# genomematt/xenomapper

Measured on AMD Instinct MI355X. Metric: read-pairs/sec classified, higher is better.
Workload: dtype int32; 1 GPU; configs[1]: 50000000 PE 2x150 pairs/GPU, AS/XS, liberal, HBM-resident; pairs_per_gpu=50000000, step=xm_classify_compact_dev: classify+count, scan, scatter (3 launches)

## Files before the change

### xenomapper_amd/csrc/xm_api.hip

```cpp
#include <hip/hip_runtime.h>
#include <stdint.h>
#include <stdio.h>
#include <stdlib.h>
#include <string.h>

#include <dlfcn.h>

#include <string>
#include <vector>

#include <rccl/rccl.h>

#include "xm_kernels.h"
#include "xm_pinned.h"

struct TimedSpan {
    int kernel;
    hipEvent_t start, stop;
};

namespace {

enum Scratch {
    S_COL0, S_COL1, S_COL2, S_COL3,
// ... 123 lines not shown
        launch();
    }
    return check_launch(ctx, what);
}

int drain_spans(xm_ctx *ctx)
{
    for (auto &sp : ctx->spans) {
        XM_HIP(ctx, hipEventSynchronize(sp.stop));
        float ms = 0.f;
        XM_HIP(ctx, hipEventElapsedTime(&ms, sp.start, sp.stop));
        ctx->acc_ms[sp.kernel] += (double)ms;
        ctx->acc_launches[sp.kernel] += 1;
        ctx->free_events.push_back(sp.start);
        ctx->free_events.push_back(sp.stop);
    }
    ctx->spans.clear();
    return XM_OK;
}

const size_t COUNTS_REP_BYTES = (XM_COUNT_REPLICAS * 64 + 8) * sizeof(uint64_t);
const size_t PART_TOT_BYTES = (size_t)XM_PART_REPLICAS * 8 * XM_PART_STRIDE * sizeof(uint32_t);

void reset_count_state(xm_ctx *ctx, hipStream_t st)
{
    (void)hipMemsetAsync(ctx->d_counts_rep, 0, COUNTS_REP_BYTES, st);
    (void)hipMemsetAsync(ctx->d_part_tot, 0, PART_TOT_BYTES, st);
}

void free_workspace(xm_ctx *ctx)
{
    if (ctx->d_gran_counts) (void)hipFree(ctx->d_gran_counts);
    if (ctx->d_gran_off) (void)hipFree(ctx->d_gran_off);
    if (ctx->d_counts_rep) (void)hipFree(ctx->d_counts_rep);
    if (ctx->d_part_tot) (void)hipFree(ctx->d_part_tot);
    if (ctx->ws_event) (void)hipEventDestroy(ctx->ws_event);
}

bool bad_mode(int mode) { return mode < XM_MODE_SE || mode > XM_MODE_PE_CONSERVATIVE; }

bool wrong_device(const xm_ctx *ctx)
{
    int cur = -1;
    return hipGetDevice(&cur) != hipSuccess || cur != ctx->device;
}

bool bad_call(const xm_ctx *ctx, int mode, uint64_t n) { return !ctx || bad_mode(mode) || n > XM_MAX_RECORDS; }
bool bad_dev_call(const xm_ctx *ctx, int mode, uint64_t n) { return bad_call(ctx, mode, n) || wrong_device(ctx); }

template <typename... P>
bool misaligned(uintptr_t mask, P... p) { return ((... | (uintptr_t)p) & mask) != 0; }

bool bad_totals(const uint64_t *offsets, const uint64_t *counts) { return !offsets || !counts || misaligned(7u, offsets, counts); }

bool capturing(hipStream_t st)
{
    hipStreamCaptureStatus cs = hipStreamCaptureStatusNone;
    if (hipStreamIsCapturing(st, &cs) != hipSuccess) { (void)hipGetLastError(); return false; }
    return cs != hipStreamCaptureStatusNone;
}

int order_workspace(xm_ctx *ctx, hipStream_t st)
{
    if (capturing(st)) return XM_OK;
    if (ctx->ws_released) {
        XM_HIP(ctx, hipStreamWaitEvent(st, ctx->ws_event, 0));
        ctx->ws_released = false;
    } else if (ctx->ws_used && ctx->ws_stream != st && !capturing(ctx->ws_stream)) {
        XM_HIP(ctx, hipEventRecord(ctx->ws_event, ctx->ws_stream));
        XM_HIP(ctx, hipStreamWaitEvent(st, ctx->ws_event, 0));
    }
    ctx->ws_stream = st;
    ctx->ws_used = true;
    return XM_OK;
}


template <typename T>
struct ScoreCols {
    const T *as1, *xs1, *as2, *xs2;
    const uint64_t *unit_bits;
    T min_score;
    static constexpr bool chunkable = true;
    static const char *kernel_name(bool counting)
    {
        if (sizeof(T) == sizeof(int32_t)) return counting ? "classify_kernel<int32, counts>" : "classify_kernel<int32>";
        return counting ? "classify_kernel<f64, counts>" : "classify_kernel<f64>";
    }
    bool missing() const { return !as1 || !xs1 || !as2 || !xs2 || !unit_bits; }
    bool misplaced() const { return misaligned(4 * sizeof(T) - 1, as1, xs1, as2, xs2) || misaligned(7u, unit_bits); }
    void classify(hipStream_t st, int mode, uint64_t n, uint8_t *code_out, const xm::CountPlan *cp) const
    {
        xm::launch_classify<T>(st, mode, n, as1, xs1, as2, xs2, unit_bits, min_score, code_out, cp);
    }
};

struct PackedCols {
    xm::CigCols s1, s2;
    const uint64_t *unit_bits;
    int32_t min_score_floor;
    uint32_t *range_flag;
    static constexpr bool chunkable = false;
    static const char *kernel_name(bool) { return "classify_cigp_kernel"; }
    bool missing() const
    {
        return !s1.nm || !s1.cnt || !s1.tile || !s1.ops || !s1.xs || !s2.nm || !s2.cnt || !s2.tile || !s2.ops || !s2.xs || !unit_bits;
    }
    bool misplaced() const
    {
        return misaligned(15u, s1.nm, s1.xs, s2.nm, s2.xs) || misaligned(7u, unit_bits) ||
               misaligned(3u, s1.cnt, s2.cnt, s1.tile, s2.tile, s1.ops, s2.ops, range_flag);
    }
    void classify(hipStream_t st, int mode, uint64_t n, uint8_t *code_out, const xm::CountPlan *cp) const
    {
        xm::launch_classify_cigp(st, mode, n, s1, s2, unit_bits, min_score_floor, code_out, range_flag, *cp);
    }
};


template <typename T>
int classify_dev(xm_ctx *ctx, hipStream_t st, int mode, uint64_t n, const ScoreCols<T> &in, uint8_t *code_out)
{
    if (bad_dev_call(ctx, mode, n)) return XM_ERR_INVALID_ARG;
    if (n == 0) return XM_OK;
    if (in.missing() || !code_out) return XM_ERR_INVALID_ARG;
    if (in.misplaced() || misaligned(3u, code_out)) return XM_ERR_INVALID_ARG;
    return timed_launch(ctx, st, XM_K_CLASSIFY, in.kernel_name(false), [&] { in.classify(st, mode, n, code_out, nullptr); });
}

int compact_tail(xm_ctx *ctx, hipStream_t st, int mode, uint64_t n, const uint8_t *code, const xm::CountPlan &cp,
                 uint32_t *idx_out, uint64_t *bin_offsets, uint64_t *counts, const xm::ListOut *lists = nullptr)
{
    const bool from_bins4 = cp.bins4 != nullptr;
    uint64_t *bin_totals = ctx->d_counts_rep + XM_COUNT_REPLICAS * 64;
    int rc = timed_launch(ctx, st, XM_K_SCAN, "scan_kernel", [&] {
        xm::launch_scan(st, cp, ctx->d_gran_off, bin_totals, counts);
    });
    if (rc == XM_OK)
        rc = timed_launch(ctx, st, XM_K_SCATTER, "scatter_kernel", [&] {
            xm::launch_scatter(st, cp.plan, mode, n, from_bins4 ? cp.bins4 : code, from_bins4, cp.gran_counts, ctx->d_gran_off,
                               bin_totals, bin_offsets, idx_out, ctx->d_part_tot, lists, cp.gran0, cp.gran1);
        });
    if (rc != XM_OK) reset_count_state(ctx, st);
    return rc;
}

xm::CountPlan count_plan(xm_ctx *ctx, uint64_t n)
{
    xm::CountPlan cp;
    cp.plan = xm::plan_granules(n);
    cp.gran_counts = ctx->d_gran_counts;
    cp.counts_rep = ctx->d_counts_rep;
    cp.part_tot = ctx->d_part_tot;
    return cp;
}

int empty_compact(xm_ctx *ctx, hipStream_t st, uint64_t *bin_offsets, uint64_t *counts)
{
    XM_HIP(ctx, hipMemsetAsync(counts, 0, 64 * sizeof(uint64_t), st));
    XM_HIP(ctx, hipMemsetAsync(bin_offsets, 0, 8 * sizeof(uint64_t), st));
    return XM_OK;
}


struct FusedDest {
    bool six_lists;
    uint32_t *flat;
    uint32_t *const *six;
    uint32_t *state6;
    uint64_t capacity;
};
FusedDest flat_list(uint32_t *idx_out) { return {false, idx_out, nullptr, nullptr, 0}; }
FusedDest six_lists(uint32_t *const idx_out[6], uint32_t *idx_state6, uint64_t cap) { return {true, nullptr, idx_out, idx_state6, cap}; }

int list_out(const FusedDest &to, xm::ListOut &lo)
{
    if (!to.six) return XM_ERR_INVALID_ARG;
    for (int b = 0; b < 6; ++b) {
        if (!to.six[b] || misaligned(3u, to.six[b])) return XM_ERR_INVALID_ARG;
        lo.p[b] = to.six[b];
    }
    if (misaligned(3u, to.state6)) return XM_ERR_INVALID_ARG;
    lo.p[6] = to.state6;
    lo.cap = to.capacity > 0xFFFFFFFFull ? 0xFFFFFFFFu : (uint32_t)to.capacity;
    return XM_OK;
}

uint32_t place_chunk_granules(void)
{
    const char *e = getenv("XM_PLACE_CHUNK_PARTS");
    const long v = e && *e ? strtol(e, nullptr, 10) : 0;
    return (uint32_t)(v < 0 ? 0 : v > 2048 ? 2048 : v) * (uint32_t)XM_PART_GRAN;
}

template <typename In>
int place_steps(xm_ctx *ctx, hipStream_t st, int mode, uint64_t n, const In &in, xm::CountPlan &cp, uint8_t *code_out,
                uint32_t *idx_out, const xm::ListOut *lists, uint64_t *totals, uint64_t *counts, bool may_chunk)
{
    const uint32_t n_gran = cp.plan.n_gran, chunk = may_chunk ? place_chunk_granules() : 0u;
    const bool chunked = chunk != 0u && n_gran > 2u * chunk;
    int rc;
    for (uint32_t g0 = 0; g0 < n_gran; g0 += chunked ? chunk : n_gran) {
        if (chunked) {
            cp.gran0 = g0;
            cp.gran1 = n_gran - g0 > chunk ? g0 + chunk : n_gran;
        }
        rc = timed_launch(ctx, st, XM_K_CLASSIFY, in.kernel_name(true), [&] { in.classify(st, mode, n, code_out, &cp); });
        if (rc != XM_OK) {
            if (g0) reset_count_state(ctx, st);
            return rc;
        }
        if ((rc = compact_tail(ctx, st, mode, n, code_out, cp, idx_out, totals, counts, lists)) != XM_OK) return rc;
    }
    return XM_OK;
}

template <typename In>
int fused_step(xm_ctx *ctx, hipStream_t st, int mode, uint64_t n, const In &in, uint8_t *code_out, uint8_t *bins4,
               const FusedDest &to, uint64_t *totals, uint64_t *counts)
{
    if (bad_dev_call(ctx, mode, n)) return XM_ERR_INVALID_ARG;
    if (bad_totals(totals, counts)) return XM_ERR_INVALID_ARG;
    xm::ListOut lo;
    int rc;
    if (to.six_lists && (rc = list_out(to, lo)) != XM_OK) return rc;
    if (n == 0) return empty_compact(ctx, st, totals, counts);
    if (in.missing() || (!code_out && !bins4) || (!to.six_lists && !to.flat)) return XM_ERR_INVALID_ARG;
    if (in.misplaced() || misaligned(15u, code_out, bins4) || misaligned(3u, to.flat)) return XM_ERR_INVALID_ARG;
    xm::CountPlan cp = count_plan(ctx, n);
    cp.bins4 = bins4;
    if ((rc = order_workspace(ctx, st)) != XM_OK) return rc;
    return place_steps(ctx, st, mode, n, in, cp, code_out, to.flat, to.six_lists ? &lo : nullptr, totals, counts,
                       In::chunkable && to.six_lists);
}


template <typename T>
int classify_runs(xm_ctx *ctx, hipStream_t st, int mode, uint64_t n, const ScoreCols<T> &in,
                  uint16_t *runs16, uint16_t *gran_counts, uint64_t *n_out, uint64_t *counts)
{
    if (bad_dev_call(ctx, mode, n)) return XM_ERR_INVALID_ARG;
    if (bad_totals(n_out, counts)) return XM_ERR_INVALID_ARG;
    if (n == 0) return empty_compact(ctx, st, n_out, counts);
    if (in.missing() || !runs16 || !gran_counts) return XM_ERR_INVALID_ARG;
    if (in.misplaced() || misaligned(15u, runs16, gran_counts)) return XM_ERR_INVALID_ARG;
    const xm::RunsOut ro = {runs16, gran_counts, ctx->d_counts_rep};
    int rc;
    if ((rc = order_workspace(ctx, st)) != XM_OK) return rc;
    rc = timed_launch(ctx, st, XM_K_CLASSIFY, "classify_runs_kernel", [&] {
        xm::launch_classify_runs<T>(st, mode, n, in.as1, in.xs1, in.as2, in.xs2, in.unit_bits, in.min_score, ro);
    });
    if (rc != XM_OK) return rc;
    rc = timed_launch(ctx, st, XM_K_SCAN, "runs_finish_kernel", [&] {
        xm::launch_runs_finish(st, mode, ctx->d_counts_rep, counts, n_out);
    });
    if (rc != XM_OK) reset_count_state(ctx, st);
    return rc;
}


template <typename T>
int upload_score_cols(xm_ctx *ctx, uint64_t n, const ScoreCols<T> &host, ScoreCols<T> &dev)
{
    const size_t col_bytes = (size_t)n * sizeof(T);
    const size_t bits_bytes = (size_t)((n + 63) / 64) * 8;
    const T *src[4] = {host.as1, host.xs1, host.as2, host.xs2};
    int rc;
    for (int c = 0; c < 4; ++c) {
        if ((rc = ensure_scratch(ctx, S_COL0 + c, col_bytes)) != XM_OK) return rc;
        XM_HIP(ctx, hipMemcpy(ctx->d_scratch[S_COL0 + c], src[c], col_bytes, hipMemcpyHostToDevice));
    }
    if ((rc = ensure_scratch(ctx, S_BITS, bits_bytes)) != XM_OK) return rc;
    XM_HIP(ctx, hipMemcpy(ctx->d_scratch[S_BITS], host.unit_bits, bits_bytes, hipMemcpyHostToDevice));
    dev = {(const T *)ctx->d_scratch[S_COL0], (const T *)ctx->d_scratch[S_COL1], (const T *)ctx->d_scratch[S_COL2],
           (const T *)ctx->d_scratch[S_COL3], (const uint64_t *)ctx->d_scratch[S_BITS], host.min_score};
    return XM_OK;
}

int ensure_code_scratch(xm_ctx *ctx, uint64_t n, bool want_bytes, uint8_t *&d_code, uint8_t *&d_bins4)
{
    const int rc = ensure_scratch(ctx, S_CODE, want_bytes ? (size_t)n + 16 : (size_t)XM_BINS4_BYTES(n));
    d_code = want_bytes ? (uint8_t *)ctx->d_scratch[S_CODE] : nullptr;
    d_bins4 = want_bytes ? nullptr : (uint8_t *)ctx->d_scratch[S_CODE];
    return rc;
}

int fetch_results(xm_ctx *ctx, uint64_t n, int n_lists, int word0, const uint32_t *const d_list[], uint32_t *const list[],
                  uint64_t cap, uint8_t *code_out, uint64_t totals[8], uint64_t counts[64])
{
    uint64_t host[72];
    XM_HIP(ctx, hipMemcpy(host, ctx->d_scratch[S_TOTALS], sizeof host, hipMemcpyDeviceToHost));
    memcpy(totals, host, 8 * sizeof(uint64_t));
    if (counts) memcpy(counts, host + 8, 64 * sizeof(uint64_t));
    for (int b = 0; b < n_lists; ++b) {
        const uint64_t k = host[word0 + b] < cap ? host[word0 + b] : cap;
        if (k) XM_HIP(ctx, hipMemcpy(list[b], d_list[b], (size_t)k * 4, hipMemcpyDeviceToHost));
    }
    if (code_out) XM_HIP(ctx, hipMemcpy(code_out, ctx->d_scratch[S_CODE], (size_t)n, hipMemcpyDeviceToHost));
    return XM_OK;
}

int fetch_compact_results(xm_ctx *ctx, uint64_t n, uint8_t *code_out, uint32_t *idx_out, uint64_t bin_offsets[8], uint64_t counts[64])
{
    const uint32_t *d_idx = (const uint32_t *)ctx->d_scratch[S_IDX];
    return fetch_results(ctx, n, 1, 7, &d_idx, &idx_out, n, code_out, bin_offsets, counts);
}

int counts_only_tail(xm_ctx *ctx, const xm::CountPlan &cp, uint64_t *d_counts)
{
    xm::launch_scan(nullptr, cp, ctx->d_gran_off, ctx->d_counts_rep + XM_COUNT_REPLICAS * 64, d_counts);
    const int rc = check_launch(ctx, "scan_kernel");
    if (rc != XM_OK) reset_count_state(ctx, nullptr);
    else (void)hipMemsetAsync(ctx->d_part_tot, 0, PART_TOT_BYTES, nullptr);
// ... 834 lines not shown
```

### xenomapper_amd/csrc/xm_kernels.h

```cpp
#pragma once
#include <hip/hip_runtime.h>
#include <stdint.h>

#include "../../include/xenomapper_hip.h"

#define XM_BLOCK 256
#define XM_GRAN 2048
#define XM_MAX_GRANULES ((uint32_t)((0xFFFFF000ull + XM_GRAN - 1) / XM_GRAN))
#define XM_PART_GRAN 1024u
#define XM_PART_STRIDE 2112u
#define XM_PART_REPLICAS 64u
#define XM_COUNT_REPLICAS 64u
#define XM_CLASSIFY_BLOCK 512
#ifndef XM_CIGAR_BLOCK
#define XM_CIGAR_BLOCK 256
#endif
#define XM_CIGP_BLOCK 512
#ifndef XM_SCATTER_WAVES
#define XM_SCATTER_WAVES 1048576u
#endif
#define XM_CLASSIFY_NT true

namespace xm {

struct GranPlan {
    uint32_t n_gran;
    uint32_t gran_stride;
};

struct CountPlan {
    GranPlan plan = {0, 0};
    uint32_t *gran_counts = nullptr;
    uint32_t *part_tot = nullptr;
    uint8_t *bins4 = nullptr;
    uint64_t *counts_rep = nullptr;
    uint32_t gran0 = 0, gran1 = 0;
};

GranPlan plan_granules(uint64_t n);

struct CigCols {
    const int32_t *nm;
    const int32_t *xs;
    const uint8_t *cnt;
    const uint32_t *tile;
    const uint32_t *ops;
};

struct ListOut {
    uint32_t *p[7];
    uint32_t cap;
};

struct RunsOut {
    uint16_t *runs16;
    uint16_t *gran_counts16;
    uint64_t *counts_rep;
};
template <typename T>
void launch_classify_runs(hipStream_t st, int mode, uint64_t n, const T *as1, const T *xs1, const T *as2, const T *xs2,
                          const uint64_t *unit_bits, T m, const RunsOut &ro);
void launch_runs_finish(hipStream_t st, int mode, uint64_t *counts_rep, uint64_t *counts, uint64_t *n_out);

template <typename T>
void launch_classify(hipStream_t st, int mode, uint64_t n, const T *as1, const T *xs1, const T *as2, const T *xs2,
                     const uint64_t *unit_bits, T m, uint8_t *code, const CountPlan *cp);
void launch_classify_cigar(hipStream_t st, int mode, uint64_t n,
                           const int32_t *nm1, const uint32_t *off1, const uint32_t *ops1, const int32_t *xs1,
                           const int32_t *nm2, const uint32_t *off2, const uint32_t *ops2, const int32_t *xs2,
                           const uint64_t *unit_bits, int32_t m, uint8_t *code, uint32_t *range_flag);
void launch_classify_cigp(hipStream_t st, int mode, uint64_t n, const CigCols &s1, const CigCols &s2,
                          const uint64_t *unit_bits, int32_t m, uint8_t *code, uint32_t *range_flag, const CountPlan &cp);
void launch_hist(hipStream_t st, int mode, uint64_t n, const uint8_t *code, const CountPlan &cp);
void launch_scan(hipStream_t st, const CountPlan &cp, uint32_t *gran_off, uint64_t *bin_totals, uint64_t *counts);
void launch_scatter(hipStream_t st, const GranPlan &p, int mode, uint64_t n, const uint8_t *code, bool code_is_bins4,
                    const uint32_t *gran_counts, const uint32_t *gran_off, const uint64_t *bin_totals, uint64_t *bin_offsets,
                    uint32_t *idx_out, uint32_t *part_tot, const ListOut *lists = nullptr, uint32_t gran0 = 0, uint32_t gran1 = 0);
void launch_stream_probe(hipStream_t st, uint64_t n, const int32_t *c0, const int32_t *c1, const int32_t *c2, const int32_t *c3,
                         uint8_t *out);
void launch_mate_correlate(hipStream_t st, uint64_t n, const double *track, uint32_t m, const double *density, double *out);
void launch_cigar(hipStream_t st, uint32_t max_blocks, uint64_t n, const int32_t *nm, const uint32_t *cig_off,
                  const uint32_t *cig_oplen, int32_t *as_out, uint32_t *range_flag);

}
```

### xenomapper_amd/csrc/xm_kernels.hip

```cpp
#include <hip/hip_runtime.h>
#include <stdint.h>
#include <stdlib.h>

#include "xm_kernels.h"

namespace xm {

template <typename T>
__device__ __forceinline__ uint32_t mapping_state(T a1, T x1, T a2, T x2, T m)
{
    const bool low1 = a1 <= m;
    const bool low2 = a2 <= m;
    const bool prim = (a1 > m) && (low2 || a1 > a2);
    const bool sec  = (a2 > m) && (low1 || a2 > a1);
    const bool spec1 = (x1 == T(0)) || (a1 > x1);
    const bool spec2 = (x2 == T(0)) || (a2 > x2);
    uint32_t s = 6u;
    s = sec ? (spec2 ? 1u : 3u) : s;
    s = (a1 == a2) ? 4u : s;
    s = prim ? (spec1 ? 0u : 2u) : s;
    s = (low1 && low2) ? 5u : s;
    return s;
}

// ... 101 lines not shown

struct CountSink {
    uint32_t *gran_counts;
    uint32_t *part_tot;
    unsigned long long *counts_rep;
    uint8_t *bins4;
    uint32_t gran_stride;
    int mode;
    uint32_t blk0;
};

__device__ __forceinline__ void count_flush(uint32_t *lds, uint32_t granule, const CountSink &sink)
{
    const uint32_t lane = threadIdx.x & 63u;
    uint32_t *misc = lds + 64 * XM_HREP;
    const uint4 h0 = *reinterpret_cast<const uint4 *>(lds + lane * XM_HREP);
    const uint4 h1 = *reinterpret_cast<const uint4 *>(lds + lane * XM_HREP + 4);
    const uint32_t s = h0.x + h0.y + h0.z + h0.w + h1.x + h1.y + h1.z + h1.w;
    if (s != 0u) {
        atomicAdd(&sink.counts_rep[(granule % XM_COUNT_REPLICAS) * 64u + lane], (unsigned long long)s);
        atomicAdd(&misc[8u + bin_of_code(sink.mode, lane)], s);
    }
    lds_settle();
    if (lane < 8u) {
        const uint32_t v = misc[8u + lane];
        sink.gran_counts[(uint64_t)lane * sink.gran_stride + granule] = v;
        if (v != 0u) atomicAdd(&sink.part_tot[((granule & (XM_PART_REPLICAS - 1u)) * 8u + lane) * XM_PART_STRIDE + granule / XM_PART_GRAN], v);
    }
}

template <int BLOCK>
__device__ __forceinline__ void count_units(const uint32_t c[4], uint32_t *lds, const CountSink &sink)
{
    const uint32_t lane = threadIdx.x & 63u;
    const uint32_t rep = lane & (XM_HREP - 1u);
#pragma unroll
    for (int j = 0; j < 4; ++j) {
        const bool unit = c[j] != XM_NO_UNIT;
        if (__ballot(unit) == 0ull) continue;
        if (unit) atomicAdd(&lds[(c[j] & 63u) * XM_HREP + rep], 1u);
    }
    lds_settle();
    uint32_t arrived = 0;
    if (lane == 0u) arrived = atomicAdd(&lds[64 * XM_HREP], 1u);
    arrived = (uint32_t)__builtin_amdgcn_readfirstlane((int)arrived);
    if (arrived != (uint32_t)(BLOCK / 64 - 1)) return;
    lds_settle();
    count_flush(lds, blockIdx.x + sink.blk0, sink);
}

template <int MODE, bool HAS6>
__device__ __forceinline__ uint32_t unit_bin(uint32_t c)
{
    if (MODE == XM_MODE_SE) return c == XM_NO_UNIT ? 7u : (c & 7u);
    const uint32_t f = (c >> 3) & 7u, r = c & 7u;
    const uint32_t lo = f < r ? f : r, hi = f < r ? r : f;
    uint32_t b = lo;
    if (MODE == XM_MODE_PE_CONSERVATIVE) {
        b = (((f ^ r) & 1u) != 0u || hi == 4u) ? 4u : b;
        b = (hi == 5u) ? 5u : b;
    }
    if (HAS6) b = (hi > 5u) ? 6u : b;
    return c == XM_NO_UNIT ? 7u : b;
}

template <int MODE, bool HAS6>
__device__ __forceinline__ uint32_t unit_bin_of(uint32_t f, uint32_t r, bool unit)
{
    uint32_t b;
    if (MODE == XM_MODE_SE) {
        b = r;
    } else {
        const uint32_t lo = f < r ? f : r, hi = f < r ? r : f;
        b = lo;
        if (MODE == XM_MODE_PE_CONSERVATIVE) {
            b = (((f ^ r) & 1u) != 0u || hi == 4u) ? 4u : b;
            b = (hi == 5u) ? 5u : b;
        }
        if (HAS6) b = (hi > 5u) ? 6u : b;
    }
    return unit ? b : 7u;
}

template <typename T, bool PAIRED, int BLOCK, bool FULL, bool COUNTS, int BINMODE>
__device__ __forceinline__ void classify_finish(const T a1[4], const T x1[4], const T a2[4], const T x2[4], T m,
                                                uint32_t mb, uint32_t halo, uint32_t *last_state,
                                                uint8_t *__restrict__ code, uint64_t r0, uint64_t n,
                                                uint32_t *count_lds, const CountSink &sink)
{
    const uint32_t lane = threadIdx.x & 63u;
    const uint32_t wave = threadIdx.x >> 6;
    uint32_t s[4];
#pragma unroll
    for (int j = 0; j < 4; ++j) s[j] = mapping_state<T>(a1[j], x1[j], a2[j], x2[j], m);

    uint32_t c[4], fwd[4] = {0, 0, 0, 0};
    if (PAIRED) {
        uint32_t prev = (uint32_t)__builtin_amdgcn_update_dpp(0, (int)s[3], 0x138, 0xf, 0xf, false);
        if (lane == 63) last_state[wave] = s[3];
        __syncthreads();
        if (lane == 0) prev = (wave == 0) ? halo : last_state[wave - 1];
        c[0] = (mb & 1u) ? ((prev << 3) | s[0]) : XM_NO_UNIT;
        c[1] = (mb & 2u) ? ((s[0] << 3) | s[1]) : XM_NO_UNIT;
        c[2] = (mb & 4u) ? ((s[1] << 3) | s[2]) : XM_NO_UNIT;
        c[3] = (mb & 8u) ? ((s[2] << 3) | s[3]) : XM_NO_UNIT;
        fwd[0] = prev; fwd[1] = s[0]; fwd[2] = s[1]; fwd[3] = s[2];
    } else {
        if (COUNTS) __syncthreads();
#pragma unroll
        for (int j = 0; j < 4; ++j) c[j] = ((mb >> j) & 1u) ? s[j] : XM_NO_UNIT;
    }

    if (FULL || r0 + 4 <= n) {
        if (code != nullptr) *reinterpret_cast<uint32_t *>(code + r0) = c[0] | (c[1] << 8) | (c[2] << 16) | (c[3] << 24);
    } else {
#pragma unroll
        for (int j = 0; j < 4; ++j)
            if (code != nullptr && r0 + j < n) code[r0 + j] = (uint8_t)c[j];
    }
    if (BINMODE >= 0) {
        uint32_t nib = 0;
#pragma unroll
        for (int j = 0; j < 4; ++j) nib |= unit_bin_of<BINMODE, sizeof(T) == 8>(fwd[j], s[j], ((mb >> j) & 1u) != 0u) << (4 * j);
        reinterpret_cast<uint16_t *>(sink.bins4)[r0 >> 2] = (uint16_t)nib;
    }
    if (COUNTS) count_units<BLOCK>(c, count_lds, sink);
}

template <typename T, bool PAIRED, bool NT, int BLOCK, bool FULL>
__device__ __forceinline__ void classify_load(const T *__restrict__ as1, const T *__restrict__ xs1,
                                              const T *__restrict__ as2, const T *__restrict__ xs2,
                                              const uint8_t *__restrict__ unit_bits8, T m, uint64_t n, uint64_t wg,
                                              T a1[4], T x1[4], T a2[4], T x2[4], uint32_t &mb, uint32_t &halo)
{
    const uint64_t g = wg * BLOCK + threadIdx.x;
    const uint64_t r0 = g * 4;
    mb = 0;
    halo = 0;
    if (FULL) {
        const uint32_t wave = (uint32_t)__builtin_amdgcn_readfirstlane((int)(threadIdx.x >> 6));
        const uint32_t lane = threadIdx.x & 63u;
        const v8u32_a4 mw = *reinterpret_cast<const v8u32_a4 *>(unit_bits8 + wg * (BLOCK / 2) + wave * 32u);
        load4<T, NT, true>(as1, r0, n, a1);
        load4<T, NT, true>(xs1, r0, n, x1);
        load4<T, NT, true>(as2, r0, n, a2);
        load4<T, NT, true>(xs2, r0, n, x2);
        uint32_t d = mw[0];
#pragma unroll
        for (uint32_t k = 1; k < 8u; ++k) d = ((lane >> 3) == k) ? mw[k] : d;
        mb = (d >> ((lane & 7u) * 4u)) & 0xFu;
        if (PAIRED && wave == 0u) {
            if (wg == 0) {
                if (lane == 0u) mb &= ~1u;
            } else if (mw[0] & 1u) {
                const uint64_t h = wg * (BLOCK * 4) - 1;
                halo = mapping_state<T>(as1[h], xs1[h], as2[h], xs2[h], m);
            }
        }
    } else {
        if (r0 < n) mb = (uint32_t)(unit_bits8[g >> 1] >> ((g & 1u) * 4u)) & 0xFu;
        load4<T, NT, false>(as1, r0, n, a1);
        load4<T, NT, false>(xs1, r0, n, x1);
        load4<T, NT, false>(as2, r0, n, a2);
        load4<T, NT, false>(xs2, r0, n, x2);
        if (r0 + 4 > n) mb &= (r0 < n) ? ((1u << (uint32_t)(n - r0)) - 1u) : 0u;
        if (PAIRED && threadIdx.x == 0) {
            if (r0 == 0) {
                mb &= ~1u;
            } else if (mb & 1u) {
                const uint64_t h = r0 - 1;
                halo = mapping_state<T>(as1[h], xs1[h], as2[h], xs2[h], m);
            }
        }
    }
}

template <typename T, bool PAIRED, bool NT, int BLOCK, bool FULL, bool COUNTS, int BINMODE>
__device__ __forceinline__ void classify_body(const T *__restrict__ as1, const T *__restrict__ xs1,
                                              const T *__restrict__ as2, const T *__restrict__ xs2,
                                              const uint8_t *__restrict__ unit_bits8, T m,
                                              uint8_t *__restrict__ code, uint64_t n, uint32_t *last_state,
                                              uint32_t *count_lds, const CountSink &sink)
{
    const uint64_t wg = (uint64_t)blockIdx.x + sink.blk0;
    const uint64_t r0 = (wg * BLOCK + threadIdx.x) * 4;
    T a1[4], x1[4], a2[4], x2[4];
    uint32_t mb, halo;
    classify_load<T, PAIRED, NT, BLOCK, FULL>(as1, xs1, as2, xs2, unit_bits8, m, n, wg, a1, x1, a2, x2, mb, halo);
    classify_finish<T, PAIRED, BLOCK, FULL, COUNTS, BINMODE>(a1, x1, a2, x2, m, mb, halo, last_state, code, r0, n, count_lds, sink);
}

template <int BLOCK>
__device__ __forceinline__ void count_lds_clear(uint32_t *count_lds)
{
    for (uint32_t k = threadIdx.x; k < (uint32_t)XM_COUNT_LDS_WORDS; k += BLOCK) count_lds[k] = 0;
}

template <typename T, bool PAIRED, bool NT, int BLOCK, bool COUNTS, int BINMODE>
__global__ void __launch_bounds__(BLOCK)
classify_kernel(const T *__restrict__ as1, const T *__restrict__ xs1,
                const T *__restrict__ as2, const T *__restrict__ xs2,
                const uint8_t *__restrict__ unit_bits8, T m,
                uint8_t *__restrict__ code, uint64_t n, CountSink sink)
{
    __shared__ uint32_t last_state[BLOCK / 64];
    __shared__ __attribute__((aligned(16))) uint32_t count_lds[COUNTS ? XM_COUNT_LDS_WORDS : 4];
    if (COUNTS) count_lds_clear<BLOCK>(count_lds);
    if (((uint64_t)blockIdx.x + sink.blk0 + 1) * (BLOCK * 4) <= n)
        classify_body<T, PAIRED, NT, BLOCK, true, COUNTS, BINMODE>(as1, xs1, as2, xs2, unit_bits8, m, code, n, last_state, count_lds, sink);
    else
        classify_body<T, PAIRED, NT, BLOCK, false, COUNTS, BINMODE>(as1, xs1, as2, xs2, unit_bits8, m, code, n, last_state, count_lds, sink);
}


__device__ __attribute__((noinline)) uint4 load_codes16_tail(const uint8_t *__restrict__ code, uint64_t base, uint64_t n)
{
    uint32_t w[4];
    for (int k = 0; k < 4; ++k) {
        uint32_t acc = 0;
        for (int j = 0; j < 4; ++j) {
            const uint64_t i = base + 4 * k + j;
            const uint32_t c = (i < n) ? (uint32_t)code[i] : XM_NO_UNIT;
            acc |= c << (8 * j);
        }
        w[k] = acc;
    }
    return make_uint4(w[0], w[1], w[2], w[3]);
}

__device__ __forceinline__ void load_codes16(const uint8_t *__restrict__ code, uint64_t base, uint64_t n,
                                             uint32_t w[4])
{
    uint4 v;
    if (base + 16 <= n) v = *reinterpret_cast<const uint4 *>(code + base);
    else v = load_codes16_tail(code, base, n);
    w[0] = v.x; w[1] = v.y; w[2] = v.z; w[3] = v.w;
}

__device__ __attribute__((noinline)) uint32_t load_codes4_tail(const uint8_t *__restrict__ code, uint64_t base, uint64_t n)
{
    uint32_t acc = 0;
    for (int j = 0; j < 4; ++j) {
        const uint64_t i = base + j;
        const uint32_t c = (i < n) ? (uint32_t)code[i] : XM_NO_UNIT;
        acc |= c << (8 * j);
    }
    return acc;
}

__global__ void __launch_bounds__(XM_BLOCK)
hist_kernel(const uint8_t *__restrict__ code, uint64_t n, uint32_t n_gran, CountSink sink)
{
    __shared__ __attribute__((aligned(16))) uint32_t lds_all[XM_BLOCK / 64][XM_COUNT_LDS_WORDS];
    const uint32_t lane = threadIdx.x & 63u, wave = threadIdx.x >> 6;
    uint32_t *lds = lds_all[wave];
    const uint32_t g = blockIdx.x * (XM_BLOCK / 64) + wave;
    if (g >= n_gran) return;
    for (uint32_t k = lane; k < (uint32_t)XM_COUNT_LDS_WORDS; k += 64u) lds[k] = 0;

    constexpr int TILES = XM_GRAN / 1024;
    const uint64_t rec0 = (uint64_t)g * XM_GRAN;
    uint32_t w[TILES][4];
#pragma unroll
    for (int k = 0; k < TILES; ++k) load_codes16(code, rec0 + (uint64_t)k * 1024u + lane * 16u, n, w[k]);
    lds_settle();

    const uint32_t rep = lane & (XM_HREP - 1u);
    uint32_t common = w[0][0] & 0xFFu;
    if (common == XM_NO_UNIT) common = (w[0][0] >> 8) & 0xFFu;
    common = (uint32_t)__builtin_amdgcn_readfirstlane((int)common);
    uint32_t n_common = 0;
#pragma unroll
    for (int k = 0; k < TILES; ++k) {
#pragma unroll
        for (int j = 0; j < 16; ++j) {
            const uint32_t c = (w[k][j >> 2] >> (8 * (j & 3))) & 0xFFu;
            const bool unit = c != XM_NO_UNIT;
            if (__ballot(unit) == 0ull) continue;
            const bool same = unit && c == common;
            n_common += same ? 1u : 0u;
            if (unit && !same) atomicAdd(&lds[(c & 63u) * XM_HREP + rep], 1u);
        }
    }
    if (n_common) atomicAdd(&lds[(common & 63u) * XM_HREP + rep], n_common);
    lds_settle();
    count_flush(lds, g, sink);
}

#define XM_SCAN_THREADS 1024
__device__ __forceinline__ unsigned long long block_sum_1024(unsigned long long v, unsigned long long *wsum)
{
    v += __shfl_xor(v, 1, 64);  v += __shfl_xor(v, 2, 64);  v += __shfl_xor(v, 4, 64);
    v += __shfl_xor(v, 8, 64);  v += __shfl_xor(v, 16, 64); v += __shfl_xor(v, 32, 64);
    if ((threadIdx.x & 63u) == 0u) wsum[threadIdx.x >> 6] = v;
// ... 1160 lines not shown
    classify_finish<int32_t, PAIRED, BLOCK, FULL, COUNTS, BINMODE>(a1, x1, a2, x2, m, mb, halo, last_state, code, r0, n,
                                                                   count_lds, sink);
}

template <bool PAIRED, int BLOCK, bool COUNTS, int BINMODE>
__global__ void __launch_bounds__(BLOCK)
classify_cigp_kernel(const CigCols s1, const CigCols s2, const uint8_t *__restrict__ unit_bits8, int32_t m,
                     uint8_t *__restrict__ code, uint64_t n, uint32_t n_tiles, uint32_t *__restrict__ range_flag, CountSink sink)
{
    static_assert(!COUNTS || BLOCK * 4 == XM_GRAN, "the counting workgroup is one granule");
    __shared__ uint32_t last_state[BLOCK / 64];
    __shared__ __attribute__((aligned(16))) uint32_t cig_table[BLOCK / 64][XM_CIG_WAVE_OPS + 8];
    __shared__ __attribute__((aligned(16))) uint32_t count_lds[COUNTS ? XM_COUNT_LDS_WORDS : 4];
    uint32_t *cig_T = cig_table[threadIdx.x >> 6];
    if (COUNTS) count_lds_clear<BLOCK>(count_lds);
    if (((uint64_t)blockIdx.x + 1) * (BLOCK * 4) <= n)
        classify_cigp_body<PAIRED, BLOCK, true, COUNTS, BINMODE>(s1, s2, unit_bits8, m, code, n, n_tiles, range_flag, last_state,
                                                                 cig_T, count_lds, sink);
    else
        classify_cigp_body<PAIRED, BLOCK, false, COUNTS, BINMODE>(s1, s2, unit_bits8, m, code, n, n_tiles, range_flag, last_state,
                                                                  cig_T, count_lds, sink);
}

#define XM_CORR_T 256
#define XM_CORR_M 2048
__global__ void __launch_bounds__(XM_CORR_T)
mate_correlate_kernel(const double *__restrict__ track, uint64_t n, const double *__restrict__ density, uint32_t m,
                      double *__restrict__ out)
{
#pragma clang fp contract(off)
    __shared__ double tile[XM_CORR_T + XM_CORR_M];
    const uint32_t t = threadIdx.x;
    const uint64_t i0 = (uint64_t)blockIdx.x * XM_CORR_T, i = i0 + t;
    const uint64_t left = (i < n) ? n - i : 0;
    double acc = 0.0;
    for (uint32_t j0 = 0; j0 < m; j0 += XM_CORR_M) {
        const uint32_t mm = (m - j0 < XM_CORR_M) ? m - j0 : XM_CORR_M;
        __syncthreads();
        for (uint32_t k = t; k < XM_CORR_T + mm; k += XM_CORR_T) {
            const uint64_t p = i0 + j0 + k;
            tile[k] = (p < n) ? track[p] : 0.0;
        }
        __syncthreads();
        const uint32_t lim = (left > j0) ? (uint32_t)((left - j0 < mm) ? left - j0 : mm) : 0u;
        if (__ballot(lim != mm) == 0ull) {
            for (uint32_t j = 0; j < mm; ++j) {
                const double prod = tile[t + j] * density[j0 + j];
                acc = acc + prod;
            }
        } else {
            for (uint32_t j = 0; j < mm; ++j) {
                const double prod = tile[t + j] * density[j0 + j];
                const double s = acc + prod;
                acc = (j < lim) ? s : acc;
            }
        }
    }
    if (i < n) out[i] = (track[i] == 1.0) ? 1.0 : acc;
}

__global__ void __launch_bounds__(XM_CLASSIFY_BLOCK)
stream_probe_kernel(const v4i32 *__restrict__ c0, const v4i32 *__restrict__ c1, const v4i32 *__restrict__ c2,
                    const v4i32 *__restrict__ c3, uint16_t *__restrict__ out, uint64_t n_groups)
{
    const uint64_t g = (uint64_t)blockIdx.x * XM_CLASSIFY_BLOCK + threadIdx.x;
    if (g >= n_groups) return;
    const v4i32 a = __builtin_nontemporal_load(c0 + g), b = __builtin_nontemporal_load(c1 + g);
    const v4i32 c = __builtin_nontemporal_load(c2 + g), d = __builtin_nontemporal_load(c3 + g);
    const v4i32 x = a ^ b ^ c ^ d;
    out[g] = (uint16_t)(x.x ^ x.y ^ x.z ^ x.w);
}

void launch_stream_probe(hipStream_t st, uint64_t n, const int32_t *c0, const int32_t *c1, const int32_t *c2, const int32_t *c3,
                         uint8_t *out)
{
    const uint64_t n_groups = n / 4;
    const uint32_t grid = (uint32_t)((n_groups + XM_CLASSIFY_BLOCK - 1) / XM_CLASSIFY_BLOCK);
    if (grid == 0) return;
    XM_LAUNCH(stream_probe_kernel, grid, XM_CLASSIFY_BLOCK, st, reinterpret_cast<const v4i32 *>(c0), reinterpret_cast<const v4i32 *>(c1),
                                                            reinterpret_cast<const v4i32 *>(c2), reinterpret_cast<const v4i32 *>(c3),
                                                            reinterpret_cast<uint16_t *>(out), n_groups);
}

static_assert(XM_CLASSIFY_BLOCK * 4 == XM_GRAN, "the counting classify workgroup is one granule");

GranPlan plan_granules(uint64_t n)
{
    GranPlan p;
    uint64_t g = (n + XM_GRAN - 1) / XM_GRAN;
    if (g == 0) g = 1;
    p.n_gran = (uint32_t)g;
    p.gran_stride = (p.n_gran + 63u) & ~63u;
    return p;
}

static CountSink make_sink(const CountPlan *cp, int mode)
{
    CountSink s;
    s.gran_counts = cp ? cp->gran_counts : nullptr;
    s.part_tot = cp ? cp->part_tot : nullptr;
    s.counts_rep = cp ? reinterpret_cast<unsigned long long *>(cp->counts_rep) : nullptr;
    s.bins4 = cp ? cp->bins4 : nullptr;
    s.gran_stride = cp ? cp->plan.gran_stride : 0u;
    s.mode = mode;
    s.blk0 = cp ? cp->gran0 : 0u;
    return s;
}

template <typename T>
void launch_classify(hipStream_t st, int mode, uint64_t n, const T *as1, const T *xs1, const T *as2, const T *xs2,
                     const uint64_t *unit_bits, T m, uint8_t *code, const CountPlan *cp)
{
    const uint64_t per_block = (uint64_t)XM_CLASSIFY_BLOCK * 4;
    static_assert(XM_CLASSIFY_BLOCK * 4 == XM_GRAN, "a counting workgroup is a granule: CountPlan's chunk is in both");
    const uint32_t all = (uint32_t)((n + per_block - 1) / per_block);
    const uint32_t grid = (cp && cp->gran1) ? cp->gran1 - cp->gran0 : all;
    const uint8_t *bits8 = reinterpret_cast<const uint8_t *>(unit_bits);
    const CountSink sink = make_sink(cp, mode);
    const bool paired = mode != XM_MODE_SE;
#define XM_LAUNCH_CLS(P, C, B) XM_LAUNCH((classify_kernel<T, P, XM_CLASSIFY_NT, XM_CLASSIFY_BLOCK, C, B>), grid, XM_CLASSIFY_BLOCK, st, as1, xs1, as2, xs2, bits8, m, code, n, sink)
    if (cp && cp->bins4) {
        if (mode == XM_MODE_SE) XM_LAUNCH_CLS(false, true, XM_MODE_SE);
        else if (mode == XM_MODE_PE_LIBERAL) XM_LAUNCH_CLS(true, true, XM_MODE_PE_LIBERAL);
        else XM_LAUNCH_CLS(true, true, XM_MODE_PE_CONSERVATIVE);
    }
    else if (cp) { if (paired) XM_LAUNCH_CLS(true, true, -1); else XM_LAUNCH_CLS(false, true, -1); }
    else         { if (paired) XM_LAUNCH_CLS(true, false, -1); else XM_LAUNCH_CLS(false, false, -1); }
#undef XM_LAUNCH_CLS
}

template void launch_classify<int32_t>(hipStream_t, int, uint64_t, const int32_t *, const int32_t *, const int32_t *, const int32_t *,
                                       const uint64_t *, int32_t, uint8_t *, const CountPlan *);
template void launch_classify<double>(hipStream_t, int, uint64_t, const double *, const double *, const double *, const double *,
                                      const uint64_t *, double, uint8_t *, const CountPlan *);

template <typename T>
void launch_classify_runs(hipStream_t st, int mode, uint64_t n, const T *as1, const T *xs1, const T *as2, const T *xs2,
                          const uint64_t *unit_bits, T m, const RunsOut &ro)
{
    const uint64_t per_block = (uint64_t)XM_CLASSIFY_BLOCK * 4;
    const uint32_t grid = (uint32_t)((n + per_block - 1) / per_block);
    const uint8_t *bits8 = reinterpret_cast<const uint8_t *>(unit_bits);
    RunsSink rs;
    rs.runs16 = ro.runs16;
    rs.gran_counts16 = ro.gran_counts16;
    rs.counts_rep = reinterpret_cast<unsigned long long *>(ro.counts_rep);
#define XM_LAUNCH_RUNS(P, B) XM_LAUNCH((classify_runs_kernel<T, P, XM_CLASSIFY_NT, XM_CLASSIFY_BLOCK, B>), grid, XM_CLASSIFY_BLOCK, st, as1, xs1, as2, xs2, bits8, m, n, rs)
    if (mode == XM_MODE_SE) XM_LAUNCH_RUNS(false, XM_MODE_SE);
    else if (mode == XM_MODE_PE_LIBERAL) XM_LAUNCH_RUNS(true, XM_MODE_PE_LIBERAL);
    else XM_LAUNCH_RUNS(true, XM_MODE_PE_CONSERVATIVE);
#undef XM_LAUNCH_RUNS
}

template void launch_classify_runs<int32_t>(hipStream_t, int, uint64_t, const int32_t *, const int32_t *, const int32_t *,
                                            const int32_t *, const uint64_t *, int32_t, const RunsOut &);
template void launch_classify_runs<double>(hipStream_t, int, uint64_t, const double *, const double *, const double *,
                                           const double *, const uint64_t *, double, const RunsOut &);

void launch_runs_finish(hipStream_t st, int mode, uint64_t *counts_rep, uint64_t *counts, uint64_t *n_out)
{
    XM_LAUNCH(runs_finish_kernel, 1, 256, st, reinterpret_cast<unsigned long long *>(counts_rep),
                                          reinterpret_cast<unsigned long long *>(counts),
                                          reinterpret_cast<unsigned long long *>(n_out), mode);
}

void launch_classify_cigar(hipStream_t st, int mode, uint64_t n,
                           const int32_t *nm1, const uint32_t *off1, const uint32_t *ops1, const int32_t *xs1,
                           const int32_t *nm2, const uint32_t *off2, const uint32_t *ops2, const int32_t *xs2,
                           const uint64_t *unit_bits, int32_t m, uint8_t *code, uint32_t *range_flag)
{
    const uint64_t per_block = (uint64_t)XM_CIGAR_BLOCK * 4;
    const uint32_t grid = (uint32_t)((n + per_block - 1) / per_block);
    const uint8_t *bits8 = reinterpret_cast<const uint8_t *>(unit_bits);
    if (mode == XM_MODE_SE)
        XM_LAUNCH((classify_cigar_kernel<false, XM_CIGAR_BLOCK>), grid, XM_CIGAR_BLOCK, st, nm1, off1, ops1, xs1, nm2, off2, ops2, xs2, bits8, m, code, n, range_flag);
    else
        XM_LAUNCH((classify_cigar_kernel<true, XM_CIGAR_BLOCK>), grid, XM_CIGAR_BLOCK, st, nm1, off1, ops1, xs1, nm2, off2, ops2, xs2, bits8, m, code, n, range_flag);
}

void launch_classify_cigp(hipStream_t st, int mode, uint64_t n, const CigCols &s1, const CigCols &s2,
                          const uint64_t *unit_bits, int32_t m, uint8_t *code, uint32_t *range_flag, const CountPlan &cp)
{
    const uint64_t per_block = (uint64_t)XM_CIGP_BLOCK * 4;
    const uint32_t grid = (uint32_t)((n + per_block - 1) / per_block);
    const uint32_t n_tiles = (uint32_t)((n + 255) / 256);
    const uint8_t *bits8 = reinterpret_cast<const uint8_t *>(unit_bits);
    const CountSink sink = make_sink(&cp, mode);
#define XM_LAUNCH_CIGP(P, B) XM_LAUNCH((classify_cigp_kernel<P, XM_CIGP_BLOCK, true, B>), grid, XM_CIGP_BLOCK, st, s1, s2, bits8, m, code, n, n_tiles, range_flag, sink)
    if (cp.bins4) {
        if (mode == XM_MODE_SE) XM_LAUNCH_CIGP(false, XM_MODE_SE);
        else if (mode == XM_MODE_PE_LIBERAL) XM_LAUNCH_CIGP(true, XM_MODE_PE_LIBERAL);
        else XM_LAUNCH_CIGP(true, XM_MODE_PE_CONSERVATIVE);
    } else {
        if (mode == XM_MODE_SE) XM_LAUNCH_CIGP(false, -1); else XM_LAUNCH_CIGP(true, -1);
    }
#undef XM_LAUNCH_CIGP
}

void launch_hist(hipStream_t st, int mode, uint64_t n, const uint8_t *code, const CountPlan &cp)
{
    const uint32_t grid = (cp.plan.n_gran + (XM_BLOCK / 64) - 1) / (XM_BLOCK / 64);
    XM_LAUNCH(hist_kernel, grid, XM_BLOCK, st, code, n, cp.plan.n_gran, make_sink(&cp, mode));
}

void launch_scan(hipStream_t st, const CountPlan &cp, uint32_t *gran_off, uint64_t *bin_totals, uint64_t *counts)
{
    const uint32_t n_parts = (cp.plan.n_gran + XM_PART_GRAN - 1) / XM_PART_GRAN;
    unsigned long long *bt = reinterpret_cast<unsigned long long *>(bin_totals);
    unsigned long long *rep = reinterpret_cast<unsigned long long *>(cp.counts_rep);
    unsigned long long *cnt = reinterpret_cast<unsigned long long *>(counts);
    const uint32_t part0 = cp.gran1 ? cp.gran0 / XM_PART_GRAN : 0u;
    const uint32_t part1 = cp.gran1 ? (cp.gran1 + XM_PART_GRAN - 1) / XM_PART_GRAN : n_parts;
    XM_LAUNCH(scan_kernel, dim3(part1 - part0, 8), XM_SCAN_THREADS, st, cp.gran_counts, cp.gran1 ? cp.gran1 : cp.plan.n_gran, cp.plan.gran_stride,
                                                                   cp.part_tot, gran_off, bt, rep, cnt, part0, n_parts);
}

static uint32_t scatter_waves()
{
    const char *e = getenv("XM_SCATTER_WAVES");
    const long v = e && *e ? strtol(e, nullptr, 10) : 0;
    return v >= 1 && v < (long)XM_SCATTER_WAVES ? (uint32_t)v : (uint32_t)XM_SCATTER_WAVES;
}

void launch_scatter(hipStream_t st, const GranPlan &p, int mode, uint64_t n, const uint8_t *code, bool code_is_bins4,
                    const uint32_t *gran_counts, const uint32_t *gran_off, const uint64_t *bin_totals, uint64_t *bin_offsets,
                    uint32_t *idx_out, uint32_t *part_tot, const ListOut *lists, uint32_t gran0, uint32_t gran1)
{
    const unsigned long long *bt = reinterpret_cast<const unsigned long long *>(bin_totals);
    unsigned long long *bo = reinterpret_cast<unsigned long long *>(bin_offsets);
    const uint32_t g_first = gran1 ? gran0 : 0u, g_end = gran1 ? gran1 : p.n_gran, span = g_end - g_first;
    const uint32_t last = g_end == p.n_gran ? 1u : 0u;
    const uint32_t max_waves = scatter_waves();
    const uint32_t gran_per_wave = (span + max_waves - 1u) / max_waves;
    const bool multi = gran_per_wave > 1u;
    const uint32_t n_waves = multi ? (span + gran_per_wave - 1u) / gran_per_wave : span;
    const uint32_t grid = (n_waves + (XM_BLOCK / 64) - 1) / (XM_BLOCK / 64);
    const bool wide = n > (1ull << 30);
    const bool stage = mode == XM_MODE_SE;
    const ListOut lo = lists ? *lists : ListOut{{nullptr, nullptr, nullptr, nullptr, nullptr, nullptr, nullptr}, 0u};
#define XM_LAUNCH_SCT(W, NIB, STG, L, M) XM_LAUNCH((scatter_kernel<XM_GRAN / 256, W, NIB, STG, L, M>), grid, XM_BLOCK, st, code, n, mode, g_end, p.gran_stride, gran_counts, gran_off, bt, bo, idx_out, part_tot, lo, gran_per_wave, g_first, last)
#define XM_LAUNCH_SCT0(W, NIB, STG, L) do { if (multi) XM_LAUNCH_SCT(W, NIB, STG, L, true); else XM_LAUNCH_SCT(W, NIB, STG, L, false); } while (0)
#define XM_LAUNCH_SCT1(W, NIB, STG) do { if (lists) XM_LAUNCH_SCT0(W, NIB, STG, true); else XM_LAUNCH_SCT0(W, NIB, STG, false); } while (0)
#define XM_LAUNCH_SCT2(W, NIB) do { if (stage) XM_LAUNCH_SCT1(W, NIB, true); else XM_LAUNCH_SCT1(W, NIB, false); } while (0)
    if (code_is_bins4) { if (wide) XM_LAUNCH_SCT2(true, true); else XM_LAUNCH_SCT2(false, true); }
    else               { if (wide) XM_LAUNCH_SCT2(true, false); else XM_LAUNCH_SCT2(false, false); }
#undef XM_LAUNCH_SCT2
#undef XM_LAUNCH_SCT1
#undef XM_LAUNCH_SCT0
#undef XM_LAUNCH_SCT
}

void launch_mate_correlate(hipStream_t st, uint64_t n, const double *track, uint32_t m, const double *density, double *out)
{
    const uint32_t grid = (uint32_t)((n + XM_CORR_T - 1) / XM_CORR_T);
    XM_LAUNCH(mate_correlate_kernel, grid, XM_CORR_T, st, track, n, density, m, out);
}

void launch_cigar(hipStream_t st, uint32_t max_blocks, uint64_t n, const int32_t *nm, const uint32_t *cig_off,
                  const uint32_t *cig_oplen, int32_t *as_out, uint32_t *range_flag)
{
    uint64_t blocks = (n + XM_BLOCK - 1) / XM_BLOCK;
    if (blocks > max_blocks) blocks = max_blocks;
    if (blocks == 0) blocks = 1;
    XM_LAUNCH(cigar_kernel, (uint32_t)blocks, XM_BLOCK, st, n, nm, cig_off, cig_oplen, as_out, range_flag);
}

}
```

Before: 149.9 billion read-pairs/s.

## Add row-major per-granule bin counts via wave ballots for paired flat compaction

Adds a paired-mode counting path in the classify kernel. Each wave computes per-bin counts with ballots and popcounts instead of the previous per-bin histogram path, and the block writes its eight bin counts contiguously per granule (row layout) with part-total atomics. A matching scan_rows_kernel reads that row layout. The aim is to cut LDS atomic traffic and strided count stores in the classify stage, at the cost of strided reads in the scan and an extra block-wide barrier.

```diff
diff --git a/xenomapper_amd/csrc/xm_api.hip b/xenomapper_amd/csrc/xm_api.hip
--- a/xenomapper_amd/csrc/xm_api.hip
+++ b/xenomapper_amd/csrc/xm_api.hip
@@ -229,6 +229,7 @@
     const uint64_t *unit_bits;
     T min_score;
     static constexpr bool chunkable = true;
+    static constexpr bool row_counts = true;
     static const char *kernel_name(bool counting)
     {
         if (sizeof(T) == sizeof(int32_t)) return counting ? "classify_kernel<int32, counts>" : "classify_kernel<int32>";
@@ -248,6 +249,7 @@
     int32_t min_score_floor;
     uint32_t *range_flag;
     static constexpr bool chunkable = false;
+    static constexpr bool row_counts = false;
     static const char *kernel_name(bool) { return "classify_cigp_kernel"; }
     bool missing() const
     {
@@ -376,6 +378,7 @@
     if (in.misplaced() || misaligned(15u, code_out, bins4) || misaligned(3u, to.flat)) return XM_ERR_INVALID_ARG;
     xm::CountPlan cp = count_plan(ctx, n);
     cp.bins4 = bins4;
+    cp.rows = In::row_counts && mode != XM_MODE_SE && !to.six_lists;
     if ((rc = order_workspace(ctx, st)) != XM_OK) return rc;
     return place_steps(ctx, st, mode, n, in, cp, code_out, to.flat, to.six_lists ? &lo : nullptr, totals, counts,
                        In::chunkable && to.six_lists);
diff --git a/xenomapper_amd/csrc/xm_kernels.h b/xenomapper_amd/csrc/xm_kernels.h
--- a/xenomapper_amd/csrc/xm_kernels.h
+++ b/xenomapper_amd/csrc/xm_kernels.h
@@ -35,6 +35,7 @@
     uint8_t *bins4 = nullptr;
     uint64_t *counts_rep = nullptr;
     uint32_t gran0 = 0, gran1 = 0;
+    bool rows = false;
 };
 
 GranPlan plan_granules(uint64_t n);
diff --git a/xenomapper_amd/csrc/xm_kernels.hip b/xenomapper_amd/csrc/xm_kernels.hip
--- a/xenomapper_amd/csrc/xm_kernels.hip
+++ b/xenomapper_amd/csrc/xm_kernels.hip
@@ -207,12 +207,39 @@
     return unit ? b : 7u;
 }
 
-template <typename T, bool PAIRED, int BLOCK, bool FULL, bool COUNTS, int BINMODE>
+#define XM_ROWS_WCNT_AT (64 * XM_HREP)
+#define XM_ROWS_LDS_WORDS (XM_ROWS_WCNT_AT + 64)
+
+template <int SLOTS, int NB>
+__device__ __forceinline__ uint32_t wave_bin_counts(const uint32_t bin[4])
+{
+    const uint32_t lane = threadIdx.x & 63u;
+    uint32_t wc = 0;
+#pragma unroll
+    for (int b = 0; b < NB; ++b) {
+        uint64_t m[4], any = 0;
+#pragma unroll
+        for (int j = 0; j < 4; ++j) {
+            m[j] = ((SLOTS >> j) & 1) ? __ballot(bin[j] == (uint32_t)b) : 0ull;
+            any |= m[j];
+        }
+        if (any == 0ull) continue;
+        uint32_t total = 0;
+#pragma unroll
+        for (int j = 0; j < 4; ++j)
+            if ((SLOTS >> j) & 1) total += (uint32_t)__builtin_popcountll(m[j]);
+        wc = (lane == (uint32_t)b) ? total : wc;
+    }
+    return wc;
+}
+
+template <typename T, bool PAIRED, int BLOCK, bool FULL, bool COUNTS, int BINMODE, int ROWS = -1>
 __device__ __forceinline__ void classify_finish(const T a1[4], const T x1[4], const T a2[4], const T x2[4], T m,
                                                 uint32_t mb, uint32_t halo, uint32_t *last_state,
                                                 uint8_t *__restrict__ code, uint64_t r0, uint64_t n,
                                                 uint32_t *count_lds, const CountSink &sink)
 {
+    static_assert(ROWS < 0 || (PAIRED && COUNTS && BLOCK == 512 && (BINMODE < 0 || BINMODE == ROWS)), "rows: paired, counting, eight waves");
     const uint32_t lane = threadIdx.x & 63u;
     const uint32_t wave = threadIdx.x >> 6;
     uint32_t s[4];
@@ -242,6 +269,43 @@
 #pragma unroll
         for (int j = 0; j < 4; ++j)
             if (code != nullptr && r0 + j < n) code[r0 + j] = (uint8_t)c[j];
+    }
+    if constexpr (ROWS >= 0) {
+        constexpr bool HAS6 = sizeof(T) == 8;
+        uint32_t bin[4];
+#pragma unroll
+        for (int j = 0; j < 4; ++j) bin[j] = unit_bin_of<ROWS, HAS6>(fwd[j], s[j], ((mb >> j) & 1u) != 0u);
+        if (BINMODE >= 0)
+            reinterpret_cast<uint16_t *>(sink.bins4)[r0 >> 2] = (uint16_t)(bin[0] | (bin[1] << 4) | (bin[2] << 8) | (bin[3] << 12));
+        {
+            const uint32_t rep = lane & (XM_HREP - 1u);
+#pragma unroll
+            for (int j = 0; j < 4; ++j) {
+                const bool unit = c[j] != XM_NO_UNIT;
+                if (__ballot(unit) == 0ull) continue;
+                if (unit) atomicAdd(&count_lds[(c[j] & 63u) * XM_HREP + rep], 1u);
+            }
+        }
+        const bool inter = __ballot((mb & 5u) != 0u) == 0ull;
+        const uint32_t wc = inter ? wave_bin_counts<0xA, HAS6 ? 7 : 6>(bin) : wave_bin_counts<0xF, HAS6 ? 7 : 6>(bin);
+        uint32_t *wave_cnt = count_lds + XM_ROWS_WCNT_AT;
+        if (lane < 8u) wave_cnt[wave * 8u + lane] = wc;
+        __syncthreads();
+        if ((uint32_t)__builtin_amdgcn_readfirstlane((int)wave) != 0u) return;
+        const uint32_t granule = blockIdx.x + sink.blk0;
+        uint32_t tot = wave_cnt[lane];
+        tot += (uint32_t)__shfl_xor((int)tot, 8, 64);
+        tot += (uint32_t)__shfl_xor((int)tot, 16, 64);
+        tot += (uint32_t)__shfl_xor((int)tot, 32, 64);
+        if (lane < 8u) {
+            sink.gran_counts[(uint64_t)granule * 8u + lane] = tot;
+            if (tot != 0u) atomicAdd(&sink.part_tot[((granule & (XM_PART_REPLICAS - 1u)) * 8u + lane) * XM_PART_STRIDE + granule / XM_PART_GRAN], tot);
+        }
+        const uint4 h0 = *reinterpret_cast<const uint4 *>(count_lds + lane * XM_HREP);
+        const uint4 h1 = *reinterpret_cast<const uint4 *>(count_lds + lane * XM_HREP + 4);
+        const uint32_t sum = h0.x + h0.y + h0.z + h0.w + h1.x + h1.y + h1.z + h1.w;
+        if (sum != 0u) atomicAdd(&sink.counts_rep[(granule % XM_COUNT_REPLICAS) * 64u + lane], (unsigned long long)sum);
+        return;
     }
     if (BINMODE >= 0) {
         uint32_t nib = 0;
@@ -300,7 +364,7 @@
     }
 }
 
-template <typename T, bool PAIRED, bool NT, int BLOCK, bool FULL, bool COUNTS, int BINMODE>
+template <typename T, bool PAIRED, bool NT, int BLOCK, bool FULL, bool COUNTS, int BINMODE, int ROWS = -1>
 __device__ __forceinline__ void classify_body(const T *__restrict__ as1, const T *__restrict__ xs1,
                                               const T *__restrict__ as2, const T *__restrict__ xs2,
                                               const uint8_t *__restrict__ unit_bits8, T m,
@@ -312,16 +376,16 @@
     T a1[4], x1[4], a2[4], x2[4];
     uint32_t mb, halo;
     classify_load<T, PAIRED, NT, BLOCK, FULL>(as1, xs1, as2, xs2, unit_bits8, m, n, wg, a1, x1, a2, x2, mb, halo);
-    classify_finish<T, PAIRED, BLOCK, FULL, COUNTS, BINMODE>(a1, x1, a2, x2, m, mb, halo, last_state, code, r0, n, count_lds, sink);
-}
-
-template <int BLOCK>
+    classify_finish<T, PAIRED, BLOCK, FULL, COUNTS, BINMODE, ROWS>(a1, x1, a2, x2, m, mb, halo, last_state, code, r0, n, count_lds, sink);
+}
+
+template <int BLOCK, int WORDS = XM_COUNT_LDS_WORDS>
 __device__ __forceinline__ void count_lds_clear(uint32_t *count_lds)
 {
-    for (uint32_t k = threadIdx.x; k < (uint32_t)XM_COUNT_LDS_WORDS; k += BLOCK) count_lds[k] = 0;
-}
-
-template <typename T, bool PAIRED, bool NT, int BLOCK, bool COUNTS, int BINMODE>
+    for (uint32_t k = threadIdx.x; k < (uint32_t)WORDS; k += BLOCK) count_lds[k] = 0;
+}
+
+template <typename T, bool PAIRED, bool NT, int BLOCK, bool COUNTS, int BINMODE, int ROWS = -1>
 __global__ void __launch_bounds__(BLOCK)
 classify_kernel(const T *__restrict__ as1, const T *__restrict__ xs1,
                 const T *__restrict__ as2, const T *__restrict__ xs2,
@@ -329,12 +393,15 @@
                 uint8_t *__restrict__ code, uint64_t n, CountSink sink)
 {
     __shared__ uint32_t last_state[BLOCK / 64];
-    __shared__ __attribute__((aligned(16))) uint32_t count_lds[COUNTS ? XM_COUNT_LDS_WORDS : 4];
-    if (COUNTS) count_lds_clear<BLOCK>(count_lds);
+    __shared__ __attribute__((aligned(16))) uint32_t count_lds[!COUNTS ? 4 : ROWS >= 0 ? XM_ROWS_LDS_WORDS : XM_COUNT_LDS_WORDS];
+    if (COUNTS) {
+        if (ROWS >= 0) count_lds_clear<BLOCK, 64 * XM_HREP>(count_lds);
+        else count_lds_clear<BLOCK>(count_lds);
+    }
     if (((uint64_t)blockIdx.x + sink.blk0 + 1) * (BLOCK * 4) <= n)
-        classify_body<T, PAIRED, NT, BLOCK, true, COUNTS, BINMODE>(as1, xs1, as2, xs2, unit_bits8, m, code, n, last_state, count_lds, sink);
+        classify_body<T, PAIRED, NT, BLOCK, true, COUNTS, BINMODE, ROWS>(as1, xs1, as2, xs2, unit_bits8, m, code, n, last_state, count_lds, sink);
     else
-        classify_body<T, PAIRED, NT, BLOCK, false, COUNTS, BINMODE>(as1, xs1, as2, xs2, unit_bits8, m, code, n, last_state, count_lds, sink);
+        classify_body<T, PAIRED, NT, BLOCK, false, COUNTS, BINMODE, ROWS>(as1, xs1, as2, xs2, unit_bits8, m, code, n, last_state, count_lds, sink);
 }
 
 
@@ -1661,6 +1728,50 @@
                                                             reinterpret_cast<uint16_t *>(out), n_groups);
 }
 
+__global__ void __launch_bounds__(XM_SCAN_THREADS)
+scan_rows_kernel(const uint32_t *__restrict__ rows, uint32_t n_gran, uint32_t gran_stride,
+                 const uint32_t *__restrict__ part_tot, uint32_t *__restrict__ gran_off,
+                 unsigned long long *__restrict__ bin_totals,
+                 unsigned long long *__restrict__ counts_rep, unsigned long long *__restrict__ counts, uint32_t part0, uint32_t n_parts)
+{
+    __shared__ unsigned long long rsum[XM_SCAN_THREADS / 64];
+    __shared__ uint32_t rtot[XM_SCAN_THREADS / 64];
+    const uint32_t p = blockIdx.x + part0, b = blockIdx.y;
+    const uint32_t t = threadIdx.x, lane = t & 63u, wave = t >> 6;
+    if (p + 1u == n_parts && t < 64u) {
+        const uint32_t slot = b * 8u + (t >> 3), part = t & 7u;
+        unsigned long long acc = 0;
+        for (uint32_t r = part; r < XM_COUNT_REPLICAS; r += 8u) {
+            acc += counts_rep[r * 64u + slot];
+            counts_rep[r * 64u + slot] = 0;
+        }
+        acc += __shfl_xor(acc, 1, 64);
+        acc += __shfl_xor(acc, 2, 64);
+        acc += __shfl_xor(acc, 4, 64);
+        if (part == 0) counts[slot] = acc;
+    }
+    const uint32_t g = p * XM_PART_GRAN + t;
+    const uint32_t x = (g < n_gran) ? rows[(uint64_t)g * 8u + b] : 0u;
+    unsigned long long part_sum = 0;
+    for (uint32_t e = t; e < p * XM_PART_REPLICAS; e += XM_SCAN_THREADS) {
+        const uint32_t r = e / p, q = e - r * p;
+        part_sum += part_tot[(r * 8u + b) * XM_PART_STRIDE + q];
+    }
+    const unsigned long long carry = block_sum_1024(part_sum, rsum);
+
+    const uint32_t incl = wave_scan_incl(x);
+    if (lane == 63u) rtot[wave] = incl;
+    __syncthreads();
+    uint32_t before_wave = 0, part_total = 0;
+    for (uint32_t w = 0; w < XM_SCAN_THREADS / 64; ++w) {
+        const uint32_t v = rtot[w];
+        before_wave += (w < wave) ? v : 0u;
+        part_total += v;
+    }
+    if (g < n_gran) gran_off[(uint64_t)b * gran_stride + g] = (uint32_t)carry + before_wave + incl - x;
+    if (p + 1u == n_parts && t == 0u) bin_totals[b] = carry + part_total;
+}
+
 static_assert(XM_CLASSIFY_BLOCK * 4 == XM_GRAN, "the counting classify workgroup is one granule");
 
 GranPlan plan_granules(uint64_t n)
@@ -1698,13 +1809,19 @@
     const CountSink sink = make_sink(cp, mode);
     const bool paired = mode != XM_MODE_SE;
 #define XM_LAUNCH_CLS(P, C, B) XM_LAUNCH((classify_kernel<T, P, XM_CLASSIFY_NT, XM_CLASSIFY_BLOCK, C, B>), grid, XM_CLASSIFY_BLOCK, st, as1, xs1, as2, xs2, bits8, m, code, n, sink)
-    if (cp && cp->bins4) {
+#define XM_LAUNCH_ROWS(B, R) XM_LAUNCH((classify_kernel<T, true, XM_CLASSIFY_NT, XM_CLASSIFY_BLOCK, true, B, R>), grid, XM_CLASSIFY_BLOCK, st, as1, xs1, as2, xs2, bits8, m, code, n, sink)
+    if (cp && cp->rows && paired) {
+        if (mode == XM_MODE_PE_LIBERAL) { if (cp->bins4) XM_LAUNCH_ROWS(XM_MODE_PE_LIBERAL, XM_MODE_PE_LIBERAL); else XM_LAUNCH_ROWS(-1, XM_MODE_PE_LIBERAL); }
+        else { if (cp->bins4) XM_LAUNCH_ROWS(XM_MODE_PE_CONSERVATIVE, XM_MODE_PE_CONSERVATIVE); else XM_LAUNCH_ROWS(-1, XM_MODE_PE_CONSERVATIVE); }
+    }
+    else if (cp && cp->bins4) {
         if (mode == XM_MODE_SE) XM_LAUNCH_CLS(false, true, XM_MODE_SE);
         else if (mode == XM_MODE_PE_LIBERAL) XM_LAUNCH_CLS(true, true, XM_MODE_PE_LIBERAL);
         else XM_LAUNCH_CLS(true, true, XM_MODE_PE_CONSERVATIVE);
     }
     else if (cp) { if (paired) XM_LAUNCH_CLS(true, true, -1); else XM_LAUNCH_CLS(false, true, -1); }
     else         { if (paired) XM_LAUNCH_CLS(true, false, -1); else XM_LAUNCH_CLS(false, false, -1); }
+#undef XM_LAUNCH_ROWS
 #undef XM_LAUNCH_CLS
 }
 
@@ -1790,8 +1907,10 @@
     unsigned long long *cnt = reinterpret_cast<unsigned long long *>(counts);
     const uint32_t part0 = cp.gran1 ? cp.gran0 / XM_PART_GRAN : 0u;
     const uint32_t part1 = cp.gran1 ? (cp.gran1 + XM_PART_GRAN - 1) / XM_PART_GRAN : n_parts;
-    XM_LAUNCH(scan_kernel, dim3(part1 - part0, 8), XM_SCAN_THREADS, st, cp.gran_counts, cp.gran1 ? cp.gran1 : cp.plan.n_gran, cp.plan.gran_stride,
-                                                                   cp.part_tot, gran_off, bt, rep, cnt, part0, n_parts);
+#define XM_LAUNCH_SCAN(K) XM_LAUNCH(K, dim3(part1 - part0, 8), XM_SCAN_THREADS, st, cp.gran_counts, cp.gran1 ? cp.gran1 : cp.plan.n_gran, cp.plan.gran_stride, \
+                                                                      cp.part_tot, gran_off, bt, rep, cnt, part0, n_parts)
+    if (cp.rows) XM_LAUNCH_SCAN(scan_rows_kernel); else XM_LAUNCH_SCAN(scan_kernel);
+#undef XM_LAUNCH_SCAN
 }
 
 static uint32_t scatter_waves()
```

Measured after the change: 150.8 billion read-pairs/s (median of 6 runs). No clear change (+0.5%).
